# lrjconan/LanczosNetwork

Hardware: NVIDIA H100
Metric: QM8 molecules/sec (forward) (higher is better)
Workload: dtype f32

## Files before the change

### include/lanczosnet_b200.h

```cpp
#ifndef LANCZOSNET_B200_H_
#define LANCZOSNET_B200_H_

#include <stdint.h>

#ifdef __cplusplus
extern "C" {
#endif

typedef void* lnb_stream_t;

#define LNB_OK 0
#define LNB_ERR_ARG (-1)
#define LNB_ERR_UNSUPPORTED (-2)

int lnb_abi_version(void);
const char* lnb_last_error(void);
int64_t lnb_launch_count(void);

int lnb_unsorted_segment_sum_forward(lnb_stream_t stream, const float* data,
                                     const int64_t* segment_ids, const int* data_shape,
                                     int num_segments, float* output);
int lnb_unsorted_segment_sum_backward(lnb_stream_t stream, const float* grad_output,
                                      const int64_t* segment_ids, const int* data_shape,
                                      int num_segments, float* grad_data);
// ... 12 lines not shown

int lnb_split_tf32(lnb_stream_t stream, const float* x, int64_t n, float* hi, float* lo);
int lnb_linear_tf32x3(lnb_stream_t stream, const float* A, const float* W_hi, const float* W_lo,
                      const float* bias, int M, int N, int K, int relu, float* C);
int lnb_linear_tf32x3_splitk(lnb_stream_t stream, const float* A, const float* W_hi, const float* W_lo,
                             const float* bias, int M, int N, int K, int relu, float* C, int splits,
                             float* workspace, int* counters);

int lnb_linear_tf32x3_grouped(lnb_stream_t stream, const float* A, const float* W_hi,
                              const float* W_lo, const float* bias, int M, int groups, int N, int K,
                              int relu, float* C);

int lnb_graph_prepare(lnb_stream_t stream, const float* L, const float* Q, int B, int N, int E1,
                      int K, float* ell_val, uint8_t* ell_idx, int32_t* ell_max, int32_t* gext,
                      int32_t* tiles, int32_t* rowmap, int32_t* nrows, int flags);
int lnb_spectral_conv_fused(lnb_stream_t stream, const float* X, const float* Q, const float* coeff,
                            const float* ell_val, const uint8_t* ell_idx, const int32_t* ell_max,
                            const int32_t* gext, const int32_t* tiles, const float* W_hi,
                            const float* W_lo, const float* bias, int B, int N, int Din, int E1,
                            int K, int S, int H, int relu, int write_pad, float* out);

int lnb_graph_prepare_sparse(lnb_stream_t stream, const int32_t* sizes, const int32_t* node_ptr,
                             const int32_t* node_feat, const int32_t* edge_ptr, const uint8_t* edges,
                             const float* V_rows, const double* inv_sqrt_deg, int B, int N, int E1,
                             int K, int flags, float* ell_val, uint8_t* ell_idx, int32_t* ell_max,
                             int32_t* gext, int32_t* tiles, int32_t* rowmap, int32_t* nrows,
                             int64_t* node_ids, uint8_t* mask, float* V, float* L_dense);

#define LNB_PACKED_HOST_TILES 2
int lnb_graph_prepare_sparse_packed(lnb_stream_t stream, const uint8_t* blob, const double* inv_sqrt_deg,
// ... 24 lines not shown
int lnb_neighbour_max(lnb_stream_t stream, const float* X, const float* ell_val, const uint8_t* ell_idx,
                      const int32_t* ell_max, int B, int N, int E1, int D, float* out ,
                      int32_t* argmax );

int lnb_embedding_rows(lnb_stream_t stream, const int64_t* idx, const float* table,
                       int64_t rows, int num_embeddings, int dim, float* out);

int lnb_ritz_power_table(lnb_stream_t stream, const float* D, int64_t rows, const int* powers,
                         int S, float* table );

int lnb_ritz_rowmap(lnb_stream_t stream, const int32_t* gext, int B, int K, int32_t* rowmap,
                    int32_t* nrows);
int lnb_ritz_filter_mlp(lnb_stream_t stream, const float* table, const int32_t* rowmap,
                        const int32_t* nrows, const float* W_hi, const float* W_lo,
                        const float* bias_all, int Rall, int L, int S, int Hd, float* coeff);

int lnb_readout(lnb_stream_t stream, const float* state, const float* W_out, const float* b_out,
                const float* w_att, const float* b_att, const uint8_t* mask, int B, int N, int H,
                int P, float* score );

int lnb_gat_attention(lnb_stream_t stream, const float* Wh, const float* bias, const float* a1,
                      const float* a2, const float* c1, const float* c2, const float* state_bias,
                      int B, int N, int E1, int heads, int F, int last, float* out);

int lnb_gat_attention_backward(lnb_stream_t stream, const float* gout, const float* Wh, const float* bias,
                               const float* a1, const float* a2, const float* c1, const float* c2,
                               const float* state_bias, int B, int N, int E1, int heads, int F, int last,
                               float* gWh, float* gpar);

int lnb_ggnn_update(lnb_stream_t stream, const float* M, const float* h, const float* ell_val,
// ... 74 lines not shown
```

### lanczosnetwork_b200/_lib.py

```python
import ctypes
import os
import threading

HERE = os.path.dirname(os.path.abspath(__file__))
LIB_PATH = os.path.join(HERE, 'liblanczosnet_b200.so')

c_f32p = ctypes.c_void_p
c_stream = ctypes.c_void_p
c_int = ctypes.c_int
c_i64 = ctypes.c_int64


class GemmDesc(ctypes.Structure):
  _fields_ = [
      ('A', ctypes.c_void_p), ('a_sb', c_i64), ('a_sz', c_i64), ('a_sm', c_i64), ('a_sk', c_i64),
      ('B', ctypes.c_void_p), ('b_sb', c_i64), ('b_sz', c_i64), ('b_sk', c_i64), ('b_sn', c_i64),
      ('C', ctypes.c_void_p), ('c_sb', c_i64), ('c_sz', c_i64), ('c_sm', c_i64), ('c_sn', c_i64),
      ('kscale', ctypes.c_void_p), ('s_sb', c_i64), ('s_sz', c_i64), ('s_sk', c_i64),
      ('bias', ctypes.c_void_p), ('bias_sz', c_i64),
      ('batch', ctypes.c_int32), ('nz', ctypes.c_int32), ('M', ctypes.c_int32),
      ('N', ctypes.c_int32), ('K', ctypes.c_int32), ('relu', ctypes.c_int32),
      ('alpha', ctypes.c_float), ('beta', ctypes.c_float),
      ('addend', ctypes.c_void_p), ('d_sb', c_i64), ('d_sz', c_i64), ('d_sm', c_i64), ('d_sn', c_i64),
  ]
# ... 25 lines not shown
        (c_int, [c_stream, c_f32p, ctypes.c_void_p, ctypes.POINTER(c_int), c_int, c_f32p]),
    'lnb_unsorted_segment_sum_backward':
        (c_int, [c_stream, c_f32p, ctypes.c_void_p, ctypes.POINTER(c_int), c_int, c_f32p]),
    'lnb_batched_gemm': (c_int, [c_stream, ctypes.POINTER(GemmDesc)]),
    'lnb_split_tf32': (c_int, [c_stream, c_f32p, c_i64, c_f32p, c_f32p]),
    'lnb_linear_tf32x3':
        (c_int, [c_stream, c_f32p, c_f32p, c_f32p, c_f32p, c_int, c_int, c_int, c_int, c_f32p]),
    'lnb_linear_tf32x3_splitk':
        (c_int, [c_stream, c_f32p, c_f32p, c_f32p, c_f32p, c_int, c_int, c_int, c_int, c_f32p, c_int,
                 c_f32p, ctypes.c_void_p]),
    'lnb_linear_tf32x3_grouped':
        (c_int, [c_stream, c_f32p, c_f32p, c_f32p, c_f32p, c_int, c_int, c_int, c_int, c_int, c_f32p]),
    'lnb_graph_prepare': (c_int, [c_stream, c_f32p, c_f32p, c_int, c_int, c_int, c_int, c_f32p,
                                  ctypes.c_void_p, ctypes.c_void_p, ctypes.c_void_p, ctypes.c_void_p,
                                  ctypes.c_void_p, ctypes.c_void_p, c_int]),
    'lnb_graph_prepare_sparse': (c_int, [c_stream] + [ctypes.c_void_p] * 7 + [c_int] * 5 +
                                 [ctypes.c_void_p] * 11),
    'lnb_graph_prepare_sparse_packed': (c_int, [c_stream] + [ctypes.c_void_p] * 2 + [c_int] * 5 +
                                        [ctypes.c_void_p] * 11),
    'lnb_spectral_conv_fused':
        (c_int, [c_stream, c_f32p, c_f32p, c_f32p, c_f32p, ctypes.c_void_p, ctypes.c_void_p,
                 ctypes.c_void_p, ctypes.c_void_p, c_f32p, c_f32p, c_f32p, c_int, c_int, c_int,
                 c_int, c_int, c_int, c_int, c_int, c_int, c_f32p]),
    'lnb_spectral_stack_forward': (c_int, [c_stream, ctypes.POINTER(SpectralStack)]),
    'lnb_sage_operators': (c_int, [c_stream, ctypes.c_void_p, c_f32p, c_int, c_int, c_int, c_int, c_f32p]),
    'lnb_sage_stack_forward': (c_int, [c_stream, ctypes.POINTER(SpectralStack), c_int]),
    'lnb_neighbour_max': (c_int, [c_stream, c_f32p, c_f32p, ctypes.c_void_p, ctypes.c_void_p, c_int, c_int,
                                  c_int, c_int, c_f32p, ctypes.c_void_p]),
    'lnb_ritz_rowmap': (c_int, [c_stream, ctypes.c_void_p, c_int, c_int, ctypes.c_void_p, ctypes.c_void_p]),
    'lnb_ritz_filter_mlp': (c_int, [c_stream, c_f32p, ctypes.c_void_p, ctypes.c_void_p, c_f32p, c_f32p,
                                    c_f32p, c_int, c_int, c_int, c_int, c_f32p]),
    'lnb_debug_set_prof': (c_int, [ctypes.c_void_p]),
    'lnb_embedding_rows': (c_int, [c_stream, ctypes.c_void_p, c_f32p, c_i64, c_int, c_int, c_f32p]),
    'lnb_ritz_power_table': (c_int, [c_stream, c_f32p, c_i64, ctypes.POINTER(c_int), c_int, c_f32p]),
    'lnb_readout': (c_int, [c_stream, c_f32p, c_f32p, c_f32p, c_f32p, c_f32p, ctypes.c_void_p,
                            c_int, c_int, c_int, c_int, c_f32p]),
    'lnb_gat_attention': (c_int, [c_stream, c_f32p, c_f32p, c_f32p, c_f32p, c_f32p, c_f32p, c_f32p,
                                  c_int, c_int, c_int, c_int, c_int, c_int, c_f32p]),
    'lnb_gat_attention_backward': (c_int, [c_stream, c_f32p, c_f32p, c_f32p, c_f32p, c_f32p, c_f32p, c_f32p,
                                           c_f32p, c_int, c_int, c_int, c_int, c_int, c_int, c_f32p, c_f32p]),
    'lnb_ggnn_update': (c_int, [c_stream, c_f32p, c_f32p, c_f32p, ctypes.c_void_p, ctypes.c_void_p, c_f32p,
                                c_f32p, c_f32p, c_int, c_int, c_int, c_int, c_int, c_f32p]),
    'lnb_sage_lstm_step': (c_int, [c_stream, c_f32p, ctypes.c_void_p, c_f32p, c_f32p, c_f32p, c_f32p, c_f32p,
                                   c_f32p, c_int, c_int, c_int, c_int, c_int, c_int, c_f32p]),
    'lnb_mpnn_update': (c_int, [c_stream, c_f32p, c_f32p, c_f32p, ctypes.c_void_p, ctypes.c_void_p, c_f32p,
                                c_f32p, c_f32p, c_int, c_int, c_int, c_int, c_int, c_f32p]),
# ... 72 lines not shown
```

### lanczosnetwork_b200/csrc/batch_prepare.cu

```cuda
#include "common.cuh"

namespace {

constexpr int BP_THREADS = 256;
constexpr int BP_EMAX = 16;
constexpr int BP_NMAX = 128;
constexpr int BP_NW = BP_NMAX / 32;

struct SparseBatchParams {
  const int32_t* sizes;
  const int32_t* node_ptr;
  const int32_t* node_feat;
  const int32_t* edge_ptr;
  const uint8_t* edges;
  const float* V_rows;
  const double* inv_sqrt_deg;
  const uint8_t* blob;
  int B, N, E1, K, flags;
  float* ell_val; uint8_t* ell_idx; int32_t* ell_max; int32_t* gext;
  int64_t* node_ids; uint8_t* mask; float* V;
  float* L;
  int32_t* rowmap; int32_t* nrows;
};

// ... 140 lines not shown
        if (m) v = __double2float_rn((scale[ch * BP_NMAX + r] * (double)m) * scale[ch * BP_NMAX + c]);
      }
      Lg[i] = v;
    }
  }
}

static int launch_sparse(lnb_stream_t stream, SparseBatchParams p, int32_t* tiles, int32_t* rowmap,
                         int32_t* nrows) {
  p.rowmap = rowmap; p.nrows = nrows;
  const size_t smem = (size_t)(p.E1 - 1) * BP_NMAX * BP_NW * 4 + (size_t)p.E1 * BP_NMAX * 8 + (size_t)p.N * p.E1 + 16;
  cudaStream_t s = (cudaStream_t)stream;
  if (smem > 48 * 1024)
    cudaFuncSetAttribute(batch_prepare_sparse_kernel, cudaFuncAttributeMaxDynamicSharedMemorySize, (int)smem);
  batch_prepare_sparse_kernel<<<p.B, BP_THREADS, smem, s>>>(p);
  if (p.blob && (p.flags & 2)) {
    lnb::count_launch(1);
  } else {
    lnb::launch_tile_assign(s, p.gext, p.B, p.K, tiles, rowmap, nrows);
    lnb::count_launch(2);
  }
  return lnb::finish_launch("graph_prepare_sparse");
}

}

extern "C" {

int lnb_graph_prepare_sparse(lnb_stream_t stream, const int32_t* sizes, const int32_t* node_ptr,
                             const int32_t* node_feat, const int32_t* edge_ptr, const uint8_t* edges,
                             const float* V_rows, const double* inv_sqrt_deg, int B, int N, int E1,
                             int K, int flags, float* ell_val, uint8_t* ell_idx, int32_t* ell_max,
                             int32_t* gext, int32_t* tiles, int32_t* rowmap, int32_t* nrows,
                             int64_t* node_ids, uint8_t* mask, float* V, float* L_dense) {
  LNB_REQUIRE(B >= 0 && N >= 1 && N <= BP_NMAX && E1 >= 2 && E1 <= BP_EMAX && K >= 1,
              "graph_prepare_sparse: bad dims B=%d N=%d E1=%d K=%d (N <= %d, 2 <= E1 <= %d)", B, N, E1,
              K, BP_NMAX, BP_EMAX);
// ... 37 lines not shown
```

### lanczosnetwork_b200/csrc/common.cuh

```cuda
#pragma once
#include <cuda_runtime.h>
#include <stdint.h>
#include <stdio.h>
#include <stdarg.h>

#include "../../include/lanczosnet_b200.h"

namespace lnb {

char* err_buf();
void set_err(const char* fmt, ...);
void count_launch(int n = 1);
unsigned long long* prof_buffer();
void set_prof_buffer(unsigned long long* p);

void launch_tile_assign(cudaStream_t s, const int32_t* gext, int B, int K, int32_t* tiles,
                        int32_t* rowmap, int32_t* nrows);

inline int finish_launch(const char* what) {
  cudaError_t e = cudaGetLastError();
  if (e != cudaSuccess) {
    set_err("%s: %s", what, cudaGetErrorString(e));
    return (int)e;
  }
  return LNB_OK;
}

#define LNB_REQUIRE(cond, ...)            \
  do {                                    \
    if (!(cond)) {                        \
      lnb::set_err(__VA_ARGS__);          \
      return LNB_ERR_ARG;                 \
// ... 13 lines not shown
```

### lanczosnetwork_b200/csrc/filter_mlp_chain.cu

```cuda
#include "tc_gemm.cuh"

namespace {

constexpr int S0MAX = 8;

struct ChainPolicy {
  static constexpr int kStagesB = 2;
  static constexpr int kStagesA = 4;
  struct Params {
    const float* table;
    const int32_t* rowmap;
    const int32_t* nrows;
    const float* W_hi;
    const float* W_lo;
    const float* bias_all;
    float* coeff;
    int Rall, L, S, Hd;
    int dbg;
  };
  static __device__ __forceinline__ bool mma0(const Params& p) { return p.S > S0MAX; }
  static __device__ __forceinline__ int first_stage(const Params& p) { return mma0(p) ? 0 : 1; }
  static __device__ __forceinline__ int steps_per_item(const Params& p) { return mma0(p) ? 4 : 2; }
  static __device__ __forceinline__ int rows(const Params& p) { return p.nrows ? __ldg(p.nrows) : p.Rall; }
  static __device__ __forceinline__ int ntile(const Params& p) { return (rows(p) + tcg::BM - 1) / tcg::BM; }
// ... 140 lines not shown
      o[4] = fmaf(y, wb.x, o[4]); o[5] = fmaf(y, wb.y, o[5]);
      o[6] = fmaf(y, wb.z, o[6]); o[7] = fmaf(y, wb.w, o[7]);
    }
    if (col + tcg::EW < p.Hd || src < 0) return;
    float* dst = p.coeff + ((int64_t)layer * p.Rall + src) * p.S;
#pragma unroll
    for (int s = 0; s < S0MAX; ++s)
      if (s < p.S) dst[s] = o[s] + b3s[s];
  }
};

__global__ void __launch_bounds__(1024)
ritz_rowmap_kernel(const int32_t* __restrict__ gext, int B, int K, int32_t* __restrict__ rowmap,
                   int32_t* __restrict__ nrows) {
  __shared__ int warp_sums[32];
  __shared__ int running;
  const int tid = threadIdx.x, lane = tid & 31, warp = tid >> 5;
  if (tid == 0) running = 0;
  __syncthreads();
  for (int b0 = 0; b0 < B; b0 += 1024) {
    const int b = b0 + tid;
    int k = (b < B) ? min(gext[b * 2 + 1], K) : 0;
    int incl = k;
#pragma unroll
    for (int o = 1; o < 32; o <<= 1) {
      const int t = __shfl_up_sync(0xffffffffu, incl, o);
      if (lane >= o) incl += t;
    }
    if (lane == 31) warp_sums[warp] = incl;
    __syncthreads();
    if (warp == 0) {
      int w = warp_sums[lane], wi = w;
#pragma unroll
      for (int o = 1; o < 32; o <<= 1) {
        const int t = __shfl_up_sync(0xffffffffu, wi, o);
        if (lane >= o) wi += t;
      }
      warp_sums[lane] = wi - w;
    }
    __syncthreads();
    const int base = running + warp_sums[warp] + incl - k;
    for (int i = 0; i < k; ++i) rowmap[base + i] = b * K + i;
    __syncthreads();
    if (tid == 1023) running = base + k;
    __syncthreads();
  }
  if (tid == 0) nrows[0] = running;
}

}

extern "C" {

int lnb_ritz_rowmap(lnb_stream_t stream, const int32_t* gext, int B, int K, int32_t* rowmap,
                    int32_t* nrows) {
  LNB_REQUIRE(gext && rowmap && nrows, "ritz_rowmap: null pointer");
  LNB_REQUIRE(B >= 0 && K >= 1, "ritz_rowmap: bad dims");
  ritz_rowmap_kernel<<<1, 1024, 0, (cudaStream_t)stream>>>(gext, B, K, rowmap, nrows);
  lnb::count_launch();
  return lnb::finish_launch("ritz_rowmap");
}

int lnb_ritz_filter_mlp(lnb_stream_t stream, const float* table, const int32_t* rowmap,
                        const int32_t* nrows, const float* W_hi, const float* W_lo,
                        const float* bias_all, int Rall, int L, int S, int Hd, float* coeff) {
  LNB_REQUIRE(table && W_hi && W_lo && bias_all && coeff, "ritz_filter_mlp: null pointer");
  LNB_REQUIRE((rowmap == nullptr) == (nrows == nullptr), "ritz_filter_mlp: rowmap and nrows go together");
  LNB_REQUIRE(Rall >= 0 && L >= 1 && S >= 1 && Hd >= 1, "ritz_filter_mlp: bad dims");
  if (S > 32 || Hd % 32 != 0 || Hd > tcg::BN) {
    lnb::set_err("ritz_filter_mlp: unsupported shape S=%d hidden=%d (needs S<=32, hidden%%32==0, hidden<=128)", S, Hd);
    return LNB_ERR_UNSUPPORTED;
  }
  if (Rall == 0) return LNB_OK;
  const size_t smem = tcg::core_smem(ChainPolicy::kStagesB, ChainPolicy::kStagesA) + 1024 + ChainPolicy::smem_bytes();
  ChainPolicy::Params p{table, rowmap, nrows, W_hi, W_lo, bias_all, coeff, Rall, L, S, Hd, tcg::debug_flags()};
  return tcg::launch<ChainPolicy>(stream, W_hi, W_lo, L * (3 * Hd + S), Hd, smem, lnb::ceil_div(Rall, tcg::BM) * L, p,
                                  "ritz_filter_mlp");
}

}
```

### lanczosnetwork_b200/csrc/spectral_conv_fused.cu

```cuda
#include "tc_gemm.cuh"

namespace {

constexpr int KMAX = 32;
constexpr int GMAX = 32;
constexpr int RMAX = 128;
constexpr int EMAX = 16;
constexpr int FR = 8;

template <bool STAGE>
__global__ void __launch_bounds__(256)
graph_prepare_kernel(const float* __restrict__ L, const float* __restrict__ Q, int N, int E1, int K,
                     float* __restrict__ ell_val, uint8_t* __restrict__ ell_idx,
                     int32_t* __restrict__ ell_max, int32_t* __restrict__ gext, int binarize) {
  extern __shared__ __align__(16) float gp_smem[];
  __shared__ int s_max[EMAX];
  __shared__ int s_ext[2];
  __shared__ uint8_t cnt_s[256 * EMAX];
  const int b = blockIdx.x, tid = threadIdx.x;
  if (tid < EMAX) s_max[tid] = 0;
  if (tid < 2) s_ext[tid] = 0;
  const int64_t per = (int64_t)N * N * E1;
  const float* Lg = L + b * per;
  if (STAGE) {
// ... 982 lines not shown

}

namespace lnb {
void launch_tile_assign(cudaStream_t s, const int32_t* gext, int B, int K, int32_t* tiles,
                        int32_t* rowmap, int32_t* nrows) {
  const size_t tbytes = ((size_t)6 * (B + 1) + 2 * SCH_NCLS) * sizeof(int32_t);
  const int tsm = tbytes <= 200 * 1024;
  if (tsm && tbytes > 40 * 1024)
    cudaFuncSetAttribute(tile_assign_kernel<true>, cudaFuncAttributeMaxDynamicSharedMemorySize, (int)tbytes);
  if (tsm)
    tile_assign_kernel<true><<<1, 1024, tbytes, s>>>(gext, B, K, tiles, tiles + B + 2, rowmap, nrows);
  else
    tile_assign_kernel<false><<<1, 1024, 0, s>>>(gext, B, K, tiles, tiles + B + 2, rowmap, nrows);
}
}

extern "C" {

int lnb_graph_prepare(lnb_stream_t stream, const float* L, const float* Q, int B, int N, int E1,
                      int K, float* ell_val, uint8_t* ell_idx, int32_t* ell_max, int32_t* gext,
                      int32_t* tiles ,
                      int32_t* rowmap, int32_t* nrows, int flags) {
  LNB_REQUIRE(L && Q && ell_val && ell_idx && ell_max && gext && tiles, "graph_prepare: null pointer");
  LNB_REQUIRE((rowmap == nullptr) == (nrows == nullptr), "graph_prepare: rowmap and nrows go together");
  LNB_REQUIRE(B >= 0 && N >= 1 && N <= 255 && E1 >= 1 && E1 <= EMAX && K >= 1,
              "graph_prepare: bad dims B=%d N=%d E1=%d K=%d", B, N, E1, K);
  if (B == 0) return LNB_OK;
  cudaStream_t s = (cudaStream_t)stream;
  const size_t lbytes = (size_t)N * N * E1 * sizeof(float);
  const int stage = lbytes <= 64 * 1024;
  if (stage) {
    if (lbytes > 40 * 1024)
      cudaFuncSetAttribute(graph_prepare_kernel<true>, cudaFuncAttributeMaxDynamicSharedMemorySize, (int)lbytes);
    graph_prepare_kernel<true><<<B, 256, lbytes, s>>>(L, Q, N, E1, K, ell_val, ell_idx, ell_max, gext,
                                                      flags & 1);
  } else {
    graph_prepare_kernel<false><<<B, 256, 0, s>>>(L, Q, N, E1, K, ell_val, ell_idx, ell_max, gext,
                                                  flags & 1);
  }
  lnb::launch_tile_assign(s, gext, B, K, tiles, rowmap, nrows);
  lnb::count_launch(2);
  return lnb::finish_launch("graph_prepare");
}

extern "C++" {
template <class Pol>
static int launch_stack(lnb_stream_t stream, const lnb_spectral_stack& d, const char* who) {
  LNB_REQUIRE((d.X || (d.node_ids && d.emb_table)) && d.Q && d.ell_val && d.ell_idx && d.ell_max &&
                  d.gext && d.tiles && d.W_hi && d.W_lo && (d.out_state || d.score) &&
                  (d.coeff || d.S == 0),
              "%s: null pointer", who);
  LNB_REQUIRE(d.B >= 0 && d.N >= 1 && d.E1 >= 1 && d.K >= 1 && d.S >= 0 && d.H >= 1 &&
                  d.num_layers >= 1 && d.num_layers <= Pol::LMAX,
              "%s: bad dims", who);
  LNB_REQUIRE(!d.score || (d.W_out && d.b_out && d.w_att && d.b_att && d.P >= 1 && d.P <= 48),
              "%s: readout needs W_out, b_out, w_att, b_att and 1 <= P <= 48", who);
  int dmax = 0;
// ... 81 lines not shown
```

### lanczosnetwork_b200/csrc/tc_gemm.cuh

```cuda
#pragma once
#include "common.cuh"
#include "sm90.cuh"
#include <stdlib.h>
#include <type_traits>

namespace tcg {

constexpr int BM = 128, BN = 128, BK = 32;
constexpr int NGROUPS = 1;
constexpr int TILE_B_BYTES = BN * BK * 4;
constexpr int STAGE_B_BYTES = 2 * TILE_B_BYTES;
constexpr int TILE_A_BYTES = BM * BK * 4;
constexpr int STAGE_A_BYTES = 2 * TILE_A_BYTES;
constexpr int EW = 16;
constexpr int PRODUCER_THREADS = 128 * NGROUPS;
constexpr int CONSUMER_WARP0 = PRODUCER_THREADS / 32;
constexpr int CONSUMER_THREADS = 256;
constexpr int THREADS = PRODUCER_THREADS + CONSUMER_THREADS;
constexpr int MAX_B_STAGES = 6, MAX_A_STAGES = 4;
__host__ __device__ constexpr int core_smem(int stages_b, int stages_a) {
  return stages_b * STAGE_B_BYTES + stages_a * STAGE_A_BYTES + 256;
}
__host__ __device__ constexpr int pass_cols(int stages_a) {
  return stages_a * STAGE_A_BYTES / (BM * 4) < BN ? stages_a * STAGE_A_BYTES / (BM * 4) : BN;
// ... 442 lines not shown
}

static unsigned long long* g_prof_mirrored = nullptr;

static int sync_prof_buffer(const char* who) {
  unsigned long long* buf = lnb::prof_buffer();
  if (buf == g_prof_mirrored) return LNB_OK;
  cudaError_t e = cudaMemcpyToSymbol(g_prof, &buf, sizeof(buf));
  if (e != cudaSuccess) { lnb::set_err("%s: %s", who, cudaGetErrorString(e)); return (int)e; }
  g_prof_mirrored = buf;
  return LNB_OK;
}

template <class Pol>
static int launch(lnb_stream_t stream, const float* W_hi, const float* W_lo, int w_rows, int w_cols,
                  size_t smem, int items, const typename Pol::Params& p, const char* who) {
  CUtensorMap map_hi, map_lo;
  int rc = make_weight_map(&map_hi, W_hi, w_rows, w_cols, who);
  if (rc != LNB_OK) return rc;
  rc = make_weight_map(&map_lo, W_lo, w_rows, w_cols, who);
  if (rc != LNB_OK) return rc;
  rc = sync_prof_buffer(who);
  if (rc != LNB_OK) return rc;
  const int skip = p.dbg & (SKIP_MMA | SKIP_TMA);
  auto kern = skip == 0                    ? tc_gemm_kernel<Pol>
              : skip == SKIP_MMA           ? tc_gemm_probe_kernel<Pol, SKIP_MMA>
              : skip == SKIP_TMA           ? tc_gemm_probe_kernel<Pol, SKIP_TMA>
                                           : tc_gemm_probe_kernel<Pol, SKIP_MMA | SKIP_TMA>;
  cudaFuncSetAttribute(kern, cudaFuncAttributeMaxDynamicSharedMemorySize, (int)smem);
  const int grid = items < sm_count() ? items : sm_count();
  kern<<<grid, THREADS, smem, (cudaStream_t)stream>>>(map_hi, map_lo, p);
  lnb::count_launch();
  return lnb::finish_launch(who);
}

}
```

### lanczosnetwork_b200/model/_common.py

```python
import os

import torch
import torch.nn as nn

from .. import _lib, ops
from ..data import check_dist
from ..spectral_conv import (GraphContext, WeightCache, graph_conv_layer,
                             ritz_filter_coefficients)


class Ragged(object):

  def __init__(self, tensor, capacity=None, bucket=4096):
    self.tensor = tensor
    rows = int(tensor.shape[0])
    self.capacity = int(capacity) if capacity is not None else max(bucket, -(-rows // bucket) * bucket)
    if rows > self.capacity:
      raise ValueError('Ragged: %d rows exceed the capacity %d' % (rows, self.capacity))

  @property
  def rows(self):
    return int(self.tensor.shape[0])

  def static_shape(self):
# ... 293 lines not shown
                         'stack kernel; call ops.graph_prepare_sparse(..., want_dense=True)')
    ctx = GraphContext(L, V, binarize)
    if prep is not None:
      ctx._prep = prep
    coeffs = table = None
    if S > 0:
      mlp = self._filter_mlp_params() if self.spectral_filter_kind == 'MLP' else None
      cur = torch.cuda.current_stream(D.device)
      side = self.__dict__.setdefault('_side_streams', {}).get(D.device.index)
      if side is None:
        side = self._side_streams[D.device.index] = torch.cuda.Stream(device=D.device)
      side.wait_stream(cur)
      with torch.cuda.stream(side):
        table = ops.ritz_power_table(D, self.long_diffusion_dist)
      table.record_stream(cur)
      gext = ctx.prep() if (mlp is not None and stack_ok and first == 0) else None
      cur.wait_stream(side)
      coeffs, table = ritz_filter_coefficients(D, self.long_diffusion_dist, mlp, self._wcache, gext,
                                               table=table)

    def layer_coeff(t):
      if S == 0:
        return None
      return coeffs[t] if coeffs is not None else table

    if node_ids is not None and not (stack_ok and first == 0):
      state = ops.embedding_rows(node_ids, self.embedding.weight)
    for t in range(first if stack_ok else nl):
      state = graph_conv_layer(state, ctx, layer_coeff(t), False, self.short_diffusion_dist, S,
                               self.filter[t].weight, self.filter[t].bias, self._wcache,
                               'filter.%d' % t, last=(t == nl - 1),
                               next_fused=(t + 1 < nl and ok[t + 1]))
    if not stack_ok:
      return self._readout(state, mask)
# ... 46 lines not shown
```

### lanczosnetwork_b200/model/lanczos_net.py

```python
import torch
import torch.nn as nn

from .. import data as data_mod
from .. import ops
from ._common import Ragged, SpectralNetBase

__all__ = ['LanczosNet']


class LanczosNet(SpectralNetBase):

  def __init__(self, config):
    super(LanczosNet, self).__init__()
    self._setup_common(config, config.dataset.num_bond_type,
                       len(config.model.long_diffusion_dist), 128)
    dims = self._build_layers()
    self.embedding = nn.Embedding(self.num_atom, self.input_dim)
    self._build_spectral_filter()
    self._build_head(dims)
    self._init_param()

  def forward(self, node_feat, L, D, V, label=None, mask=None):
    return self._forward((node_feat, L, D, V, mask), label)

# ... 34 lines not shown
  def _forward_packed_impl(self, B, N, K, blob):
    E1 = self.num_edgetype + 1
    dense = not self._sparse_stack_ok(N, E1, K)
    off_D = data_mod.packed_offsets(B, K)[3]
    D = blob[off_D:off_D + 4 * B * K].view(torch.float32).reshape(B, K)
    prep, node_ids, mask, V, L = ops.graph_prepare_sparse_packed(
        blob, B, N, E1, K, binarize=getattr(self, '_binarize_operators', False), want_dense=dense)
    return self._ritz_conv_stack(None, node_ids, L, D, V, mask, prep=prep, dims_hint=(N, E1))

  def _forward_sparse_impl(self, N, sizes, node_ptr, node_feat, edge_ptr, edges, V_rows, D):
    E1 = self.num_edgetype + 1
    K = V_rows.shape[1]
    dense = not self._sparse_stack_ok(N, E1, K)
    prep, node_ids, mask, V, L = ops.graph_prepare_sparse(
        sizes, node_ptr, node_feat, edge_ptr, edges, V_rows, N, E1,
        binarize=getattr(self, '_binarize_operators', False), want_dense=dense)
    return self._ritz_conv_stack(None, node_ids, L, D.float().contiguous(), V, mask, prep=prep,
                                 dims_hint=(N, E1))

  def _forward_sparse_eigs_impl(self, N, K, sizes, node_ptr, node_feat, edge_ptr, edges):
    D, V_rows, _ = ops.graph_eigs_sparse(sizes, node_ptr, edge_ptr, edges, N, K,
                                         num_edgetype=self.num_edgetype, rows=node_feat.shape[0])
    return self._forward_sparse_impl(N, sizes, node_ptr, node_feat, edge_ptr, edges, V_rows, D)
```

### lanczosnetwork_b200/ops.py

```python
import ctypes

import torch

from . import _lib
from ._lib import GemmDesc, SpectralStack

__all__ = [
    'bgemm', 'split_tf32', 'linear_tf32x3', 'linear_tf32x3_grouped', 'graph_prepare', 'spectral_conv_fused',
    'graph_prepare_sparse', 'graph_prepare_sparse_packed', 'graph_eigs_sparse', 'sym_eigs',
    'fused_conv_supported', 'spectral_stack_forward', 'ritz_rowmap', 'ritz_filter_mlp', 'embedding_rows', 'ritz_power_table', 'readout',
    'gat_attention', 'gat_attention_supported', 'gat_attention_backward', 'gat_attention_backward_supported',
    'sage_operators', 'neighbour_max', 'sage_lstm_step', 'sage_lstm_step_supported', 'sage_lstm_messages',
    'ggnn_update',
    'ggnn_update_supported', 'gpnn_partition_update', 'gpnn_partition_update_supported', 'mpnn_update', 'mpnn_update_supported', 'mpnn_edge_aggregate',
    'mpnn_edge_aggregate_backward', 'mpnn_edge_aggregate_supported', 'set2vec', 'set2vec_supported',
    'operator_chain', 'operator_chain_supported', 'graph_messages', 'graph_messages_supported', 'gaussian_laplacian', 'lanczos_tridiag', 'lanczos_ritz', 'tridiag_ritz', 'tridiag_powers',
    'symmetrize_filters', 'segment_sum_forward', 'segment_sum_backward', 'launch_count',
]


def _need_cuda(*tensors):
  for t in tensors:
    if t is None:
      continue
# ... 124 lines not shown
  K = w_hi.shape[1]
  N = w_hi.shape[0] // groups
  assert x.shape[1] == groups * K and w_hi.shape[0] == groups * N
  out = torch.empty((M, groups * N), device=x.device, dtype=torch.float32)
  with torch.cuda.device(x.device):
    _lib.check(_lib.load().lnb_linear_tf32x3_grouped(_stream(x), _ptr(x), _ptr(w_hi), _ptr(w_lo),
                                                     _ptr(bias), M, groups, N, K,
                                                     int(bool(relu)), _ptr(out)),
               'lnb_linear_tf32x3_grouped')
  return out


class GraphPrep(tuple):
  rowmap = None
  nrows = None


def graph_prepare(L, Q=None, binarize=False):
  if Q is None:
    Q = torch.zeros((L.shape[0], L.shape[1], 4), device=L.device, dtype=torch.float32)
  _need_cuda(L, Q)
  L, Q = _f32c(L), _f32c(Q)
  B, N, _, E1 = L.shape
  K = Q.shape[2]
  dev = L.device
  ell_val = torch.empty((B, E1, N, N), device=dev, dtype=torch.float32)
  ell_idx = torch.empty((B, E1, N, N), device=dev, dtype=torch.uint8)
  ell_max = torch.empty((B, E1), device=dev, dtype=torch.int32)
  gext = torch.empty((B, 2), device=dev, dtype=torch.int32)
  tiles = torch.empty((4 * B + 2,), device=dev, dtype=torch.int32)
  rowmap = torch.empty((B * K,), device=dev, dtype=torch.int32)
  nrows = torch.empty((1,), device=dev, dtype=torch.int32)
  with torch.cuda.device(dev):
    _lib.check(_lib.load().lnb_graph_prepare(_stream(L), _ptr(L), _ptr(Q), B, N, E1, K,
                                             _ptr(ell_val), _ptr(ell_idx), _ptr(ell_max),
                                             _ptr(gext), _ptr(tiles), _ptr(rowmap), _ptr(nrows),
                                             1 if binarize else 0),
               'lnb_graph_prepare')
  prep = GraphPrep((ell_val, ell_idx, ell_max, gext, tiles))
  prep.rowmap, prep.nrows = rowmap, nrows
  return prep


_INV_SQRT_DEG = {}


def _inv_sqrt_deg_table(device):
  key = device.index if device.index is not None else torch.cuda.current_device()
  if key not in _INV_SQRT_DEG:
    import numpy as np
    deg = np.arange(256, dtype=np.float64)
    with np.errstate(divide='ignore'):
      t = np.power(deg, -0.5)
    t[np.isinf(t)] = 0.0
    _INV_SQRT_DEG[key] = torch.from_numpy(t).to(device)
  return _INV_SQRT_DEG[key]


def graph_prepare_sparse(sizes, node_ptr, node_feat, edge_ptr, edges, V_rows, N, E1, binarize=False,
                         want_dense=False):
  _need_cuda(sizes, node_ptr, node_feat, edge_ptr, edges, V_rows)
  dev = sizes.device
  B = sizes.shape[0]
  K = V_rows.shape[1]
  assert sizes.dtype == torch.int32 and node_ptr.dtype == torch.int32 and node_feat.dtype == torch.int32
  assert edge_ptr.dtype == torch.int32 and edges.dtype == torch.uint8 and edges.shape[1] == 4
  assert V_rows.dtype == torch.float32 and V_rows.is_contiguous() and edges.is_contiguous()
  ell_val = torch.empty((B, E1, N, N), device=dev, dtype=torch.float32)
  ell_idx = torch.empty((B, E1, N, N), device=dev, dtype=torch.uint8)
  ell_max = torch.empty((B, E1), device=dev, dtype=torch.int32)
  gext = torch.empty((B, 2), device=dev, dtype=torch.int32)
  tiles = torch.empty((4 * B + 2,), device=dev, dtype=torch.int32)
  rowmap = torch.empty((B * K,), device=dev, dtype=torch.int32)
  nrows = torch.empty((1,), device=dev, dtype=torch.int32)
  node_ids = torch.empty((B, N), device=dev, dtype=torch.int64)
  mask = torch.empty((B, N), device=dev, dtype=torch.uint8)
  V = torch.empty((B, N, K), device=dev, dtype=torch.float32)
  L = torch.empty((B, N, N, E1), device=dev, dtype=torch.float32) if want_dense else None
  with torch.cuda.device(dev):
    _lib.check(_lib.load().lnb_graph_prepare_sparse(
        _stream(sizes), _ptr(sizes), _ptr(node_ptr), _ptr(node_feat), _ptr(edge_ptr), _ptr(edges),
        _ptr(V_rows), _ptr(_inv_sqrt_deg_table(dev)), B, int(N), int(E1), int(K),
        1 if binarize else 0, _ptr(ell_val), _ptr(ell_idx), _ptr(ell_max), _ptr(gext), _ptr(tiles),
        _ptr(rowmap), _ptr(nrows), _ptr(node_ids), _ptr(mask), _ptr(V), _ptr(L)),
               'lnb_graph_prepare_sparse')
  prep = GraphPrep((ell_val, ell_idx, ell_max, gext, tiles))
  prep.rowmap, prep.nrows = rowmap, nrows
  return prep, node_ids, mask, V, L


def graph_prepare_sparse_packed(blob, B, N, E1, K, binarize=False, want_dense=False, host_tiles=True):
  _need_cuda(blob)
  assert blob.dtype == torch.uint8 and blob.is_contiguous()
  dev = blob.device
  ell_val = torch.empty((B, E1, N, N), device=dev, dtype=torch.float32)
  ell_idx = torch.empty((B, E1, N, N), device=dev, dtype=torch.uint8)
  ell_max = torch.empty((B, E1), device=dev, dtype=torch.int32)
  gext = torch.empty((B, 2), device=dev, dtype=torch.int32)
  if host_tiles:
    from .data import packed_offsets, tile_segment_ints
    off_tiles = packed_offsets(B, K)[5]
    tiles = blob[off_tiles:off_tiles + 4 * tile_segment_ints(B)].view(torch.int32)
# ... 174 lines not shown
                 'lnb_sage_stack_forward')
  return state, score


def ritz_rowmap(gext, K):
  _need_cuda(gext)
  B = gext.shape[0]
  rowmap = torch.empty((B * K,), device=gext.device, dtype=torch.int32)
  nrows = torch.empty((1,), device=gext.device, dtype=torch.int32)
  with torch.cuda.device(gext.device):
    _lib.check(_lib.load().lnb_ritz_rowmap(_stream(gext), _ptr(gext), B, int(K), _ptr(rowmap),
                                           _ptr(nrows)), 'lnb_ritz_rowmap')
  return rowmap, nrows


def ritz_filter_mlp(table, w_hi, w_lo, bias_all, num_layers, rowmap=None, nrows=None):
  _need_cuda(table, w_hi, w_lo, bias_all, rowmap, nrows)
  table = _f32c(table)
  R, S = table.shape
  Hd = w_hi.shape[1]
  coeff = torch.empty((num_layers, R, S), device=table.device, dtype=torch.float32)
  with torch.cuda.device(table.device):
    _lib.check(_lib.load().lnb_ritz_filter_mlp(_stream(table), _ptr(table), _ptr(rowmap),
                                               _ptr(nrows), _ptr(w_hi), _ptr(w_lo),
                                               _ptr(bias_all), R, int(num_layers), S, Hd,
                                               _ptr(coeff)), 'lnb_ritz_filter_mlp')
  return coeff


def embedding_rows(idx, table):
  _need_cuda(idx, table)
  idx = idx.contiguous().long()
  table = _f32c(table)
  rows = idx.numel()
  out = torch.empty(tuple(idx.shape) + (table.shape[1],), device=table.device, dtype=torch.float32)
  with torch.cuda.device(table.device):
    _lib.check(_lib.load().lnb_embedding_rows(_stream(table), _ptr(idx), _ptr(table), rows,
                                              table.shape[0], table.shape[1], _ptr(out)),
               'lnb_embedding_rows')
  return out

# ... 458 lines not shown
```

### lanczosnetwork_b200/spectral_conv.py

```python
import torch

from . import ops

__all__ = ['WeightCache', 'GraphContext', 'dense', 'graph_conv_layer', 'graph_conv_layer_unfused',
           'ritz_filter_coefficients']


class WeightCache(object):

  def __init__(self):
    import threading
    self._store = {}
    self._lock = threading.Lock()
    self.bypass = False

  def _get(self, key, tag, build, sources):
    if self.bypass:
      return build()
    with self._lock:
      hit = self._store.get(key)
    if hit is None or hit[0] != tag:
      hit = (tag,) + tuple(build()) + (tuple(sources),)
      with self._lock:
        self._store[key] = hit
# ... 64 lines not shown

def dense(x2d, weight, bias, relu, cache, name):
  M, K = x2d.shape
  N = weight.shape[0]
  if K % 4 == 0:
    w_hi, w_lo = cache.split(name, weight, K)
    return ops.linear_tf32x3(x2d, w_hi, w_lo, bias, relu)
  assert K == weight.shape[1]
  out = torch.empty((M, N), device=x2d.device, dtype=torch.float32)
  w = weight.detach().contiguous()
  ops.bgemm(x2d, (0, 0, K, 1), w, (0, 0, 1, K), out, (0, 0, N, 1), 1, 1, M, N, K,
            bias=bias, relu=relu)
  return out


def ritz_filter_coefficients(D, powers, mlp_layers, cache, gext=None, table=None):
  B, K = D.shape
  S = len(powers)
  if table is None:
    table = ops.ritz_power_table(D, powers)
  if mlp_layers is None:
    return None, table
  nl = len(mlp_layers)
  flat = table.reshape(B * K, S)
  hd = mlp_layers[0][0][1].shape[0]
  if S <= 32 and hd % 32 == 0 and hd <= 128:
    w_hi, w_lo, bias_all = cache.split_mlp_chain('spectral_filter.chain', mlp_layers)
    rowmap = nrows = None
    if isinstance(gext, ops.GraphPrep):
      rowmap, nrows = gext.rowmap, gext.nrows
    elif gext is not None:
      rowmap, nrows = ops.ritz_rowmap(gext, K)
    coeff = ops.ritz_filter_mlp(flat, w_hi, w_lo, bias_all, nl, rowmap, nrows).reshape(nl, B, K, S)
    return coeff, table
  if S % 4 == 0 and hd % 4 == 0:
    h = flat
    for stage in range(4):
      ws = [mlp_layers[l][stage][1] for l in range(nl)]
      bs = [mlp_layers[l][stage][2] for l in range(nl)]
      w_hi, w_lo, bias = cache.split_stacked('spectral_filter.*.%d' % (2 * stage), ws, bs)
      if stage == 0:
        h = ops.linear_tf32x3(h, w_hi, w_lo, bias, True)
      else:
        h = ops.linear_tf32x3_grouped(h, w_hi, w_lo, bias, nl, stage < 3)
    coeff = h.reshape(B, K, nl, S).permute(2, 0, 1, 3).contiguous()
    return coeff, table
  out = []
  for params in mlp_layers:
    h = flat
    for i, (name, w, b) in enumerate(params):
      h = dense(h, w, b, i < len(params) - 1, cache, name)
    out.append(h.reshape(B, K, S))
  return torch.stack(out, dim=0), table


class GraphContext(object):

  def __init__(self, L, Qv, binarize=False):
    self.L = L
    self.Qv = Qv
    self.binarize = binarize
    self._prep = None

  def prep(self):
    if self._prep is None:
      self._prep = ops.graph_prepare(self.L, self.Qv, self.binarize)
    return self._prep


def graph_conv_layer(state, ctx, coeff, dense_filter, short_dist, num_long, weight, bias, cache,
                     name, last=True, next_fused=False):
  L, Qv = ctx.L, ctx.Qv
  B, N, Din = state.shape
  if (num_long > 0 and Qv is not None and
      ops.fused_conv_supported(N, Din, Qv.shape[2], weight.shape[0], len(short_dist), dense_filter,
                               num_long, L.shape[3])):
    w_hi, w_lo = cache.split(name, weight)
    return ops.spectral_conv_fused(state, Qv, coeff, ctx.prep(), w_hi, w_lo, bias, True,
                                   write_pad=last or not next_fused)
  return graph_conv_layer_unfused(state, L, Qv, coeff, dense_filter, short_dist, num_long, weight,
                                  bias, cache, name)
# ... 61 lines not shown
```

Before: 1.072 million.

## Defer tile assignment to a side stream overlapping the Ritz filter MLP

Graph preparation can now skip the single-CTA tile-assignment kernel and emit only the rowmap. Tile assignment then runs on a side stream concurrently with the Ritz filter MLP, which is capped to SM count minus one CTAs to leave room for it. The rowmap kernel also writes its output cooperatively across warps instead of one thread per graph looping serially. This adds stream synchronisation and a lazy tiles_pending state that later consumers must resolve, and capping the MLP grid may slow it slightly.

Measured after the change: 1.104 million, median of 6. +3.0%, better.

```diff
diff --git a/include/lanczosnet_b200.h b/include/lanczosnet_b200.h
--- a/include/lanczosnet_b200.h
+++ b/include/lanczosnet_b200.h
@@ -50,6 +50,8 @@
 int lnb_graph_prepare(lnb_stream_t stream, const float* L, const float* Q, int B, int N, int E1,
                       int K, float* ell_val, uint8_t* ell_idx, int32_t* ell_max, int32_t* gext,
                       int32_t* tiles, int32_t* rowmap, int32_t* nrows, int flags);
+#define LNB_PREP_DEFER_TILES 4
+int lnb_tile_assign(lnb_stream_t stream, const int32_t* gext, int B, int K, int32_t* tiles);
 int lnb_spectral_conv_fused(lnb_stream_t stream, const float* X, const float* Q, const float* coeff,
                             const float* ell_val, const uint8_t* ell_idx, const int32_t* ell_max,
                             const int32_t* gext, const int32_t* tiles, const float* W_hi,
@@ -104,6 +106,10 @@
 int lnb_ritz_filter_mlp(lnb_stream_t stream, const float* table, const int32_t* rowmap,
                         const int32_t* nrows, const float* W_hi, const float* W_lo,
                         const float* bias_all, int Rall, int L, int S, int Hd, float* coeff);
+int lnb_ritz_filter_mlp_ctas(lnb_stream_t stream, const float* table, const int32_t* rowmap,
+                             const int32_t* nrows, const float* W_hi, const float* W_lo,
+                             const float* bias_all, int Rall, int L, int S, int Hd, float* coeff,
+                             int ctas);
 
 int lnb_readout(lnb_stream_t stream, const float* state, const float* W_out, const float* b_out,
                 const float* w_att, const float* b_att, const uint8_t* mask, int B, int N, int H,
diff --git a/lanczosnetwork_b200/_lib.py b/lanczosnetwork_b200/_lib.py
--- a/lanczosnetwork_b200/_lib.py
+++ b/lanczosnetwork_b200/_lib.py
@@ -63,6 +63,7 @@
     'lnb_graph_prepare': (c_int, [c_stream, c_f32p, c_f32p, c_int, c_int, c_int, c_int, c_f32p,
                                   ctypes.c_void_p, ctypes.c_void_p, ctypes.c_void_p, ctypes.c_void_p,
                                   ctypes.c_void_p, ctypes.c_void_p, c_int]),
+    'lnb_tile_assign': (c_int, [c_stream, ctypes.c_void_p, c_int, c_int, ctypes.c_void_p]),
     'lnb_graph_prepare_sparse': (c_int, [c_stream] + [ctypes.c_void_p] * 7 + [c_int] * 5 +
                                  [ctypes.c_void_p] * 11),
     'lnb_graph_prepare_sparse_packed': (c_int, [c_stream] + [ctypes.c_void_p] * 2 + [c_int] * 5 +
@@ -79,6 +80,8 @@
     'lnb_ritz_rowmap': (c_int, [c_stream, ctypes.c_void_p, c_int, c_int, ctypes.c_void_p, ctypes.c_void_p]),
     'lnb_ritz_filter_mlp': (c_int, [c_stream, c_f32p, ctypes.c_void_p, ctypes.c_void_p, c_f32p, c_f32p,
                                     c_f32p, c_int, c_int, c_int, c_int, c_f32p]),
+    'lnb_ritz_filter_mlp_ctas': (c_int, [c_stream, c_f32p, ctypes.c_void_p, ctypes.c_void_p, c_f32p, c_f32p,
+                                         c_f32p, c_int, c_int, c_int, c_int, c_f32p, c_int]),
     'lnb_debug_set_prof': (c_int, [ctypes.c_void_p]),
     'lnb_embedding_rows': (c_int, [c_stream, ctypes.c_void_p, c_f32p, c_i64, c_int, c_int, c_f32p]),
     'lnb_ritz_power_table': (c_int, [c_stream, c_f32p, c_i64, ctypes.POINTER(c_int), c_int, c_f32p]),
diff --git a/lanczosnetwork_b200/csrc/batch_prepare.cu b/lanczosnetwork_b200/csrc/batch_prepare.cu
--- a/lanczosnetwork_b200/csrc/batch_prepare.cu
+++ b/lanczosnetwork_b200/csrc/batch_prepare.cu
@@ -178,13 +178,11 @@
   if (smem > 48 * 1024)
     cudaFuncSetAttribute(batch_prepare_sparse_kernel, cudaFuncAttributeMaxDynamicSharedMemorySize, (int)smem);
   batch_prepare_sparse_kernel<<<p.B, BP_THREADS, smem, s>>>(p);
-  if (p.blob && (p.flags & 2)) {
-    lnb::count_launch(1);
-  } else {
-    lnb::launch_tile_assign(s, p.gext, p.B, p.K, tiles, rowmap, nrows);
-    lnb::count_launch(2);
-  }
-  return lnb::finish_launch("graph_prepare_sparse");
+  lnb::count_launch(1);
+  if (p.blob && (p.flags & 2))
+    return lnb::finish_launch("graph_prepare_sparse");
+  return lnb::launch_tiles_or_rowmap(s, p.flags, p.gext, p.B, p.K, tiles, rowmap, nrows,
+                                     "graph_prepare_sparse");
 }
 
 }
diff --git a/lanczosnetwork_b200/csrc/common.cuh b/lanczosnetwork_b200/csrc/common.cuh
--- a/lanczosnetwork_b200/csrc/common.cuh
+++ b/lanczosnetwork_b200/csrc/common.cuh
@@ -16,6 +16,8 @@
 
 void launch_tile_assign(cudaStream_t s, const int32_t* gext, int B, int K, int32_t* tiles,
                         int32_t* rowmap, int32_t* nrows);
+int launch_tiles_or_rowmap(cudaStream_t s, int flags, const int32_t* gext, int B, int K,
+                           int32_t* tiles, int32_t* rowmap, int32_t* nrows, const char* who);
 
 inline int finish_launch(const char* what) {
   cudaError_t e = cudaGetLastError();
diff --git a/lanczosnetwork_b200/csrc/filter_mlp_chain.cu b/lanczosnetwork_b200/csrc/filter_mlp_chain.cu
--- a/lanczosnetwork_b200/csrc/filter_mlp_chain.cu
+++ b/lanczosnetwork_b200/csrc/filter_mlp_chain.cu
@@ -178,6 +178,7 @@
 ritz_rowmap_kernel(const int32_t* __restrict__ gext, int B, int K, int32_t* __restrict__ rowmap,
                    int32_t* __restrict__ nrows) {
   __shared__ int warp_sums[32];
+  __shared__ int gbase[1024], gk[1024];
   __shared__ int running;
   const int tid = threadIdx.x, lane = tid & 31, warp = tid >> 5;
   if (tid == 0) running = 0;
@@ -204,9 +205,12 @@
     }
     __syncthreads();
     const int base = running + warp_sums[warp] + incl - k;
-    for (int i = 0; i < k; ++i) rowmap[base + i] = b * K + i;
+    gbase[tid] = base;
+    gk[tid] = k;
     __syncthreads();
     if (tid == 1023) running = base + k;
+    for (int j = warp; j < 1024 && b0 + j < B; j += 32)
+      for (int i = lane; i < gk[j]; i += 32) rowmap[gbase[j] + i] = (b0 + j) * K + i;
     __syncthreads();
   }
   if (tid == 0) nrows[0] = running;
@@ -228,9 +232,17 @@
 int lnb_ritz_filter_mlp(lnb_stream_t stream, const float* table, const int32_t* rowmap,
                         const int32_t* nrows, const float* W_hi, const float* W_lo,
                         const float* bias_all, int Rall, int L, int S, int Hd, float* coeff) {
+  return lnb_ritz_filter_mlp_ctas(stream, table, rowmap, nrows, W_hi, W_lo, bias_all, Rall, L, S, Hd,
+                                  coeff, 0);
+}
+
+int lnb_ritz_filter_mlp_ctas(lnb_stream_t stream, const float* table, const int32_t* rowmap,
+                             const int32_t* nrows, const float* W_hi, const float* W_lo,
+                             const float* bias_all, int Rall, int L, int S, int Hd, float* coeff,
+                             int ctas) {
   LNB_REQUIRE(table && W_hi && W_lo && bias_all && coeff, "ritz_filter_mlp: null pointer");
   LNB_REQUIRE((rowmap == nullptr) == (nrows == nullptr), "ritz_filter_mlp: rowmap and nrows go together");
-  LNB_REQUIRE(Rall >= 0 && L >= 1 && S >= 1 && Hd >= 1, "ritz_filter_mlp: bad dims");
+  LNB_REQUIRE(Rall >= 0 && L >= 1 && S >= 1 && Hd >= 1 && ctas >= 0, "ritz_filter_mlp: bad dims");
   if (S > 32 || Hd % 32 != 0 || Hd > tcg::BN) {
     lnb::set_err("ritz_filter_mlp: unsupported shape S=%d hidden=%d (needs S<=32, hidden%%32==0, hidden<=128)", S, Hd);
     return LNB_ERR_UNSUPPORTED;
@@ -239,7 +251,7 @@
   const size_t smem = tcg::core_smem(ChainPolicy::kStagesB, ChainPolicy::kStagesA) + 1024 + ChainPolicy::smem_bytes();
   ChainPolicy::Params p{table, rowmap, nrows, W_hi, W_lo, bias_all, coeff, Rall, L, S, Hd, tcg::debug_flags()};
   return tcg::launch<ChainPolicy>(stream, W_hi, W_lo, L * (3 * Hd + S), Hd, smem, lnb::ceil_div(Rall, tcg::BM) * L, p,
-                                  "ritz_filter_mlp");
-}
-
-}
+                                  "ritz_filter_mlp", ctas);
+}
+
+}
diff --git a/lanczosnetwork_b200/csrc/spectral_conv_fused.cu b/lanczosnetwork_b200/csrc/spectral_conv_fused.cu
--- a/lanczosnetwork_b200/csrc/spectral_conv_fused.cu
+++ b/lanczosnetwork_b200/csrc/spectral_conv_fused.cu
@@ -1020,6 +1020,18 @@
   else
     tile_assign_kernel<false><<<1, 1024, 0, s>>>(gext, B, K, tiles, tiles + B + 2, rowmap, nrows);
 }
+
+int launch_tiles_or_rowmap(cudaStream_t s, int flags, const int32_t* gext, int B, int K,
+                           int32_t* tiles, int32_t* rowmap, int32_t* nrows, const char* who) {
+  if (flags & LNB_PREP_DEFER_TILES) {
+    int rc = lnb::finish_launch(who);
+    if (rc == LNB_OK && rowmap) rc = lnb_ritz_rowmap((lnb_stream_t)s, gext, B, K, rowmap, nrows);
+    return rc;
+  }
+  launch_tile_assign(s, gext, B, K, tiles, rowmap, nrows);
+  count_launch();
+  return finish_launch(who);
+}
 }
 
 extern "C" {
@@ -1045,9 +1057,17 @@
     graph_prepare_kernel<false><<<B, 256, 0, s>>>(L, Q, N, E1, K, ell_val, ell_idx, ell_max, gext,
                                                   flags & 1);
   }
-  lnb::launch_tile_assign(s, gext, B, K, tiles, rowmap, nrows);
-  lnb::count_launch(2);
-  return lnb::finish_launch("graph_prepare");
+  lnb::count_launch(1);
+  return lnb::launch_tiles_or_rowmap(s, flags, gext, B, K, tiles, rowmap, nrows, "graph_prepare");
+}
+
+int lnb_tile_assign(lnb_stream_t stream, const int32_t* gext, int B, int K, int32_t* tiles) {
+  LNB_REQUIRE(gext && tiles, "tile_assign: null pointer");
+  LNB_REQUIRE(B >= 0 && K >= 1, "tile_assign: bad dims B=%d K=%d", B, K);
+  if (B == 0) return LNB_OK;
+  lnb::launch_tile_assign((cudaStream_t)stream, gext, B, K, tiles, nullptr, nullptr);
+  lnb::count_launch();
+  return lnb::finish_launch("tile_assign");
 }
 
 extern "C++" {
diff --git a/lanczosnetwork_b200/csrc/tc_gemm.cuh b/lanczosnetwork_b200/csrc/tc_gemm.cuh
--- a/lanczosnetwork_b200/csrc/tc_gemm.cuh
+++ b/lanczosnetwork_b200/csrc/tc_gemm.cuh
@@ -480,7 +480,8 @@
 
 template <class Pol>
 static int launch(lnb_stream_t stream, const float* W_hi, const float* W_lo, int w_rows, int w_cols,
-                  size_t smem, int items, const typename Pol::Params& p, const char* who) {
+                  size_t smem, int items, const typename Pol::Params& p, const char* who,
+                  int max_ctas = 0) {
   CUtensorMap map_hi, map_lo;
   int rc = make_weight_map(&map_hi, W_hi, w_rows, w_cols, who);
   if (rc != LNB_OK) return rc;
@@ -494,7 +495,8 @@
               : skip == SKIP_TMA           ? tc_gemm_probe_kernel<Pol, SKIP_TMA>
                                            : tc_gemm_probe_kernel<Pol, SKIP_MMA | SKIP_TMA>;
   cudaFuncSetAttribute(kern, cudaFuncAttributeMaxDynamicSharedMemorySize, (int)smem);
-  const int grid = items < sm_count() ? items : sm_count();
+  int grid = items < sm_count() ? items : sm_count();
+  if (max_ctas > 0 && grid > max_ctas) grid = max_ctas;
   kern<<<grid, THREADS, smem, (cudaStream_t)stream>>>(map_hi, map_lo, p);
   lnb::count_launch();
   return lnb::finish_launch(who);
diff --git a/lanczosnetwork_b200/model/_common.py b/lanczosnetwork_b200/model/_common.py
--- a/lanczosnetwork_b200/model/_common.py
+++ b/lanczosnetwork_b200/model/_common.py
@@ -331,10 +331,17 @@
       with torch.cuda.stream(side):
         table = ops.ritz_power_table(D, self.long_diffusion_dist)
       table.record_stream(cur)
-      gext = ctx.prep() if (mlp is not None and stack_ok and first == 0) else None
+      gext = ctx.prep(defer_tiles=True) if (mlp is not None and stack_ok and first == 0) else None
       cur.wait_stream(side)
+      ctas = 0
+      if gext is not None and gext.tiles_pending:
+        side.wait_stream(cur)
+        with torch.cuda.stream(side):
+          ops.tile_assign(gext, K)
+        ctas = torch.cuda.get_device_properties(D.device).multi_processor_count - 1
       coeffs, table = ritz_filter_coefficients(D, self.long_diffusion_dist, mlp, self._wcache, gext,
-                                               table=table)
+                                               table=table, ctas=ctas)
+      cur.wait_stream(side)
 
     def layer_coeff(t):
       if S == 0:
diff --git a/lanczosnetwork_b200/model/lanczos_net.py b/lanczosnetwork_b200/model/lanczos_net.py
--- a/lanczosnetwork_b200/model/lanczos_net.py
+++ b/lanczosnetwork_b200/model/lanczos_net.py
@@ -72,7 +72,7 @@
     dense = not self._sparse_stack_ok(N, E1, K)
     prep, node_ids, mask, V, L = ops.graph_prepare_sparse(
         sizes, node_ptr, node_feat, edge_ptr, edges, V_rows, N, E1,
-        binarize=getattr(self, '_binarize_operators', False), want_dense=dense)
+        binarize=getattr(self, '_binarize_operators', False), want_dense=dense, defer_tiles=True)
     return self._ritz_conv_stack(None, node_ids, L, D.float().contiguous(), V, mask, prep=prep,
                                  dims_hint=(N, E1))
 
diff --git a/lanczosnetwork_b200/ops.py b/lanczosnetwork_b200/ops.py
--- a/lanczosnetwork_b200/ops.py
+++ b/lanczosnetwork_b200/ops.py
@@ -6,7 +6,7 @@
 from ._lib import GemmDesc, SpectralStack
 
 __all__ = [
-    'bgemm', 'split_tf32', 'linear_tf32x3', 'linear_tf32x3_grouped', 'graph_prepare', 'spectral_conv_fused',
+    'bgemm', 'split_tf32', 'linear_tf32x3', 'linear_tf32x3_grouped', 'graph_prepare', 'tile_assign', 'spectral_conv_fused',
     'graph_prepare_sparse', 'graph_prepare_sparse_packed', 'graph_eigs_sparse', 'sym_eigs',
     'fused_conv_supported', 'spectral_stack_forward', 'ritz_rowmap', 'ritz_filter_mlp', 'embedding_rows', 'ritz_power_table', 'readout',
     'gat_attention', 'gat_attention_supported', 'gat_attention_backward', 'gat_attention_backward_supported',
@@ -162,9 +162,21 @@
 class GraphPrep(tuple):
   rowmap = None
   nrows = None
-
-
-def graph_prepare(L, Q=None, binarize=False):
+  tiles_pending = False
+
+
+def tile_assign(prep, K):
+  gext, tiles = prep[3], prep[4]
+  with torch.cuda.device(gext.device):
+    _lib.check(_lib.load().lnb_tile_assign(_stream(gext), _ptr(gext), gext.shape[0], int(K), _ptr(tiles)),
+               'lnb_tile_assign')
+  prep.tiles_pending = False
+
+
+PREP_DEFER_TILES = 4
+
+
+def graph_prepare(L, Q=None, binarize=False, defer_tiles=False):
   if Q is None:
     Q = torch.zeros((L.shape[0], L.shape[1], 4), device=L.device, dtype=torch.float32)
   _need_cuda(L, Q)
@@ -183,10 +195,10 @@
     _lib.check(_lib.load().lnb_graph_prepare(_stream(L), _ptr(L), _ptr(Q), B, N, E1, K,
                                              _ptr(ell_val), _ptr(ell_idx), _ptr(ell_max),
                                              _ptr(gext), _ptr(tiles), _ptr(rowmap), _ptr(nrows),
-                                             1 if binarize else 0),
+                                             (1 if binarize else 0) | (PREP_DEFER_TILES if defer_tiles else 0)),
                'lnb_graph_prepare')
   prep = GraphPrep((ell_val, ell_idx, ell_max, gext, tiles))
-  prep.rowmap, prep.nrows = rowmap, nrows
+  prep.rowmap, prep.nrows, prep.tiles_pending = rowmap, nrows, bool(defer_tiles) and B > 0
   return prep
 
 
@@ -206,7 +218,7 @@
 
 
 def graph_prepare_sparse(sizes, node_ptr, node_feat, edge_ptr, edges, V_rows, N, E1, binarize=False,
-                         want_dense=False):
+                         want_dense=False, defer_tiles=False):
   _need_cuda(sizes, node_ptr, node_feat, edge_ptr, edges, V_rows)
   dev = sizes.device
   B = sizes.shape[0]
@@ -229,11 +241,12 @@
     _lib.check(_lib.load().lnb_graph_prepare_sparse(
         _stream(sizes), _ptr(sizes), _ptr(node_ptr), _ptr(node_feat), _ptr(edge_ptr), _ptr(edges),
         _ptr(V_rows), _ptr(_inv_sqrt_deg_table(dev)), B, int(N), int(E1), int(K),
-        1 if binarize else 0, _ptr(ell_val), _ptr(ell_idx), _ptr(ell_max), _ptr(gext), _ptr(tiles),
+        (1 if binarize else 0) | (PREP_DEFER_TILES if defer_tiles else 0), _ptr(ell_val), _ptr(ell_idx),
+        _ptr(ell_max), _ptr(gext), _ptr(tiles),
         _ptr(rowmap), _ptr(nrows), _ptr(node_ids), _ptr(mask), _ptr(V), _ptr(L)),
                'lnb_graph_prepare_sparse')
   prep = GraphPrep((ell_val, ell_idx, ell_max, gext, tiles))
-  prep.rowmap, prep.nrows = rowmap, nrows
+  prep.rowmap, prep.nrows, prep.tiles_pending = rowmap, nrows, bool(defer_tiles) and B > 0
   return prep, node_ids, mask, V, L
 
 
@@ -438,17 +451,17 @@
   return rowmap, nrows
 
 
-def ritz_filter_mlp(table, w_hi, w_lo, bias_all, num_layers, rowmap=None, nrows=None):
+def ritz_filter_mlp(table, w_hi, w_lo, bias_all, num_layers, rowmap=None, nrows=None, ctas=0):
   _need_cuda(table, w_hi, w_lo, bias_all, rowmap, nrows)
   table = _f32c(table)
   R, S = table.shape
   Hd = w_hi.shape[1]
   coeff = torch.empty((num_layers, R, S), device=table.device, dtype=torch.float32)
   with torch.cuda.device(table.device):
-    _lib.check(_lib.load().lnb_ritz_filter_mlp(_stream(table), _ptr(table), _ptr(rowmap),
-                                               _ptr(nrows), _ptr(w_hi), _ptr(w_lo),
-                                               _ptr(bias_all), R, int(num_layers), S, Hd,
-                                               _ptr(coeff)), 'lnb_ritz_filter_mlp')
+    _lib.check(_lib.load().lnb_ritz_filter_mlp_ctas(_stream(table), _ptr(table), _ptr(rowmap),
+                                                    _ptr(nrows), _ptr(w_hi), _ptr(w_lo),
+                                                    _ptr(bias_all), R, int(num_layers), S, Hd,
+                                                    _ptr(coeff), int(ctas)), 'lnb_ritz_filter_mlp')
   return coeff
 
 
diff --git a/lanczosnetwork_b200/spectral_conv.py b/lanczosnetwork_b200/spectral_conv.py
--- a/lanczosnetwork_b200/spectral_conv.py
+++ b/lanczosnetwork_b200/spectral_conv.py
@@ -102,7 +102,7 @@
   return out
 
 
-def ritz_filter_coefficients(D, powers, mlp_layers, cache, gext=None, table=None):
+def ritz_filter_coefficients(D, powers, mlp_layers, cache, gext=None, table=None, ctas=0):
   B, K = D.shape
   S = len(powers)
   if table is None:
@@ -119,7 +119,7 @@
       rowmap, nrows = gext.rowmap, gext.nrows
     elif gext is not None:
       rowmap, nrows = ops.ritz_rowmap(gext, K)
-    coeff = ops.ritz_filter_mlp(flat, w_hi, w_lo, bias_all, nl, rowmap, nrows).reshape(nl, B, K, S)
+    coeff = ops.ritz_filter_mlp(flat, w_hi, w_lo, bias_all, nl, rowmap, nrows, ctas).reshape(nl, B, K, S)
     return coeff, table
   if S % 4 == 0 and hd % 4 == 0:
     h = flat
@@ -150,9 +150,11 @@
     self.binarize = binarize
     self._prep = None
 
-  def prep(self):
+  def prep(self, defer_tiles=False):
     if self._prep is None:
-      self._prep = ops.graph_prepare(self.L, self.Qv, self.binarize)
+      self._prep = ops.graph_prepare(self.L, self.Qv, self.binarize, defer_tiles)
+    elif getattr(self._prep, 'tiles_pending', False) and not defer_tiles:
+      ops.tile_assign(self._prep, self.Qv.shape[2])
     return self._prep
 
 
```
